# nicolas1805961/Cardiac-Segmentation-Optical-flow

Measured on AMD Instinct MI355X. Metric: cine frames/sec (seg+flow) at 256x256, higher is better.
Workload: dtype f16 MFMA hi/lo split, f32 accumulate (f32-class); 1 GPU; BASELINE config 4: joint seg+flow over 256x256x30 cine slices; Generic_UNet(32 base, 6 pools) 4-flip TTA on every frame + SegFlowGaussian(video.yaml) two-chunk ED-anchored recurrence + fused label warp; image=256x256

## Files before the change

cardiac-segmentation-optical-flow_amd/cineflow/_lib.py:

```python
import ctypes
import os

_HERE = os.path.dirname(os.path.abspath(__file__))
LIB_PATH = os.environ.get("CINEFLOW_LIB") or os.path.join(_HERE, "libcineflow_hip.so")


class CineflowLibraryError(RuntimeError):
    pass


class CineflowError(RuntimeError):
    pass


P = ctypes.c_void_p
I = ctypes.c_int
L = ctypes.c_long
F = ctypes.c_float
DBL = ctypes.c_double

SIGNATURES = {
    "cf_warp_bilinear_2d": [P, P, P, I, I, I, I, P],
    "cf_vecint_2d": [P, P, P, I, I, I, I, P],
    "cf_warp_labels_2d": [P, P, P, I, I, I, I, I, P],
# ... 41 lines not shown
    "cf_crop2d": [P, P, I, I, I, I, I, I, I, P],
    "cf_pad2d": [P, P, I, I, I, I, I, I, I, P],
    "cf_tta_accumulate": [P, P, I, I, I, I, I, I, F, P],
    "cf_flip2d": [P, P, I, I, I, I, I, P],
    "cf_tile_accumulate": [P, P, P, P, I, I, I, I, I, I, I, P],
    "cf_tile_finalize": [P, P, P, P, I, I, I, P],
    "cf_tile_gather": [P, P, P, I, I, I, I, I, I, I, P],
    "cf_tile_merge": [P, P, P, P, I, I, I, I, I, I, P, I, P, I, P],
    "cf_tta_accumulate_3d": [P, P, I, I, I, I, I, I, I, I, F, P],
    "cf_flip3d": [P, P, I, I, I, I, I, I, I, P],
    "cf_tile_accumulate_3d": [P, P, P, P, I, I, I, I, I, I, I, I, I, I, P],
    "cf_argmax_channels": [P, P, I, I, I, P],
    "cf_resize3d": [P, P, I, I, I, I, I, I, I, I, I, I, P],
    "cf_cc_init": [P, P, L, P, I, P],
    "cf_cc_sweep": [P, I, I, I, P, P],
    "cf_cc_count": [P, P, L, P],
    "cf_cc_remove": [P, P, P, L, I, DBL, DBL, P],
    "cf_cc_label": [P, P, I, I, I, P, P],
    "cf_cc_sizes": [P, P, P, P, L, P, P, P, P],
    "cf_pp_confusion": [P, P, I, I, I, I, P, P, P, P, P, P, P, DBL, P, P, P, P],
    "cf_cc_apply": [P, P, L, I, I, I, P, P, P, P, P, P, DBL, P, P],
    "cf_conv2d_small_cin": [P, P, P, P, I, I, I, I, I, I, P, I, P],
    "cf_conv2d_small_cout": [P, P, P, P, P, I, I, I, I, I, P],
    "cf_nonzero_mask": [P, I, L, P, P],
    "cf_fill_holes": [P, P, P, I, I, I, I, P],
    "cf_mask_bbox": [P, I, I, I, P, P],
    "cf_spline3_resample_axis": [P, P, L, I, L, I, P],
    "cf_slab_minmax_chunks": [I, I, I, L],
    "cf_slab_minmax": [P, I, I, I, L, P, P, P],
    "cf_slab_clip_to_f32": [P, P, I, I, I, L, P, P],
    "cf_masked_moments": [P, P, L, I, F, F, P, P],
    "cf_normalize": [P, P, L, I, F, F, F, F, I, P],
    "cf_nan_to_zero": [P, L, P],
    "cf_assign_where_ge": [P, P, L, F, F, P],
    "cf_seg_outside_mask": [P, P, I, L, F, P],
    "cf_prev_stage_onehot": [P, I, I, I, P, I, I, I, P, I, P],
    "cf_ensemble_merge": [P, I, I, I, I, I, I, P, I, I, I, I, I, I, P, P, P],
    "cf_confusion_counts": [P, P, L, P, P],
    "cf_label_confusion": [P, P, L, I, P, P],
    "cf_surface_border": [P, I, I, I, I, P, P, P],
    "cf_surface_min_dist": [P, I, P, I, DBL, DBL, DBL, P, P],
    "cf_max_sum_nonneg": [P, L, P, P],
    "cf_region_stats": [P, P, L, I, P, P],
    "cf_spatial_gradient3d": [P, P, L, I, I, I, P],
    "cf_slab_abs_sum": [P, I, I, I, L, P, P],
    "cf_ssim_map": [P, P, I, I, I, DBL, DBL, DBL, P, P],
# ... 40 lines not shown
```

cardiac-segmentation-optical-flow_amd/cineflow/inference.py:

```python
import os

import numpy as np
import torch

from . import ops


def compute_steps_for_sliding_window(patch_size, image_size, step_size):
    assert all(i >= j for i, j in zip(image_size, patch_size)), "image size must be as large or larger than patch_size"
    assert 0 < step_size <= 1, "step_size must be larger than 0 and smaller or equal to 1"
    target = [i * step_size for i in patch_size]
    num_steps = [int(np.ceil((i - k) / j)) + 1 for i, j, k in zip(image_size, target, patch_size)]
    steps = []
    for dim in range(len(patch_size)):
        max_step_value = image_size[dim] - patch_size[dim]
        actual = max_step_value / (num_steps[dim] - 1) if num_steps[dim] > 1 else 99999999999
        steps.append([int(np.round(actual * i)) for i in range(num_steps[dim])])
    return steps


def get_gaussian(patch_size, sigma_scale=1.0 / 8):
    from scipy.ndimage import gaussian_filter
    tmp = np.zeros(patch_size)
    tmp[tuple(i // 2 for i in patch_size)] = 1
# ... 298 lines not shown
    key = str(dev)
    if key not in _side:
        _side[key] = torch.cuda.Stream(device=dev)
    return _side[key]


def predict_cine_slices(flow_net, seg_net, frames, ed_labels=None, do_mirroring=True, mirror_axes=(0, 1), seg_mixed_precision=False):
    T, B, _, H, W = frames.shape
    dev = frames.device
    seg_terms = 1 if seg_mixed_precision else 3
    side = None
    if TWO_STREAMS:
        side = _side_stream(dev)
        side.wait_stream(torch.cuda.current_stream(dev))
        with torch.cuda.stream(side), ops.conv_terms(seg_terms):
            probs = ensemble_predict_2d(seg_net, frames.reshape(T * B, 1, H, W), mirror_axes, do_mirroring)
            seg = ops.argmax_channels(probs).view(T, B, H, W)
    else:
        with ops.conv_terms(seg_terms):
            probs = ensemble_predict_2d(seg_net, frames.reshape(T * B, 1, H, W), mirror_axes, do_mirroring)
        seg = ops.argmax_channels(probs).view(T, B, H, W)
    flow = torch.zeros((T, B, 2, H, W), dtype=torch.float32, device=dev)
    o1, o2 = chunk_orders(T)
    ragged = len(o1) == len(o2) + 1 and len(o2) > 1 and RAGGED_CHUNKS and hasattr(flow_net, "_narrow") and not getattr(flow_net, "raft", False)
    if len(o1) == len(o2) and len(o1) > 1:
        xin = torch.cat([frames[o1], frames[o2]], dim=1)
        bf = flow_net(xin)["backward_flow"]
        for j, t in enumerate(o1[1:]):
            flow[t] = bf[j, :B]
        for j, t in enumerate(o2[1:]):
            flow[t] = bf[j, B:]
    elif ragged:
        o2p = o2 + [o2[-1]]
        xin = torch.cat([frames[o1], frames[o2p]], dim=1)
        bf = flow_net(xin, keep_from=len(o2), keep=B)["backward_flow"]
        for j, t in enumerate(o1[1:]):
            flow[t] = bf[j, :B]
        for j, t in enumerate(o2[1:]):
            flow[t] = bf[j, B:]
    else:
        for order in (o1, o2):
            if len(order) > 1:
                bf = flow_net(frames[order].contiguous())["backward_flow"]
                for j, t in enumerate(order[1:]):
                    flow[t] = bf[j]
    if side is not None:
        torch.cuda.current_stream(dev).wait_stream(side)
        probs.record_stream(torch.cuda.current_stream(dev))
        seg.record_stream(torch.cuda.current_stream(dev))
    if ed_labels is None:
        ed_labels = seg[0].contiguous()
    registered = ops.warp_labels(flow, ed_labels, flow_net.num_classes if hasattr(flow_net, "num_classes") else 4)
    return {"seg": seg, "softmax": probs.view(T, B, -1, H, W), "flow": flow, "registered": registered}
```

cardiac-segmentation-optical-flow_amd/cineflow/models.py:

```python
import copy

import numpy as np
import torch

from . import ops
from .convroute import PackedConv
from .nn import (Module, conv_norm, Conv2d, ConvTranspose2d, GroupNorm, Conv3d, ConvTranspose3d, InstanceNorm3d, ResidualLayer3D, ConvBlocks2DGroupLegacy, Encoder2D, Decoder2D, CrossAttentionLayer,
                 TransformerFlowEncoderSuccessiveNoEmb, ConvGRUCell, SpatialTransformer, VecInt)


class CorrVolume(Module):

    def __init__(self, radius, stride):
        super().__init__()
        self.radius, self.stride = radius, stride

    def forward(self, cur, prev):
        return ops.corr_volume(cur, prev, self.radius, self.stride)


class CorrBlock:

    def __init__(self, fmap1, fmap2, num_levels=4, radius=4):
        self.num_levels, self.radius = num_levels, radius
# ... 119 lines not shown
            self.query_encoder = Encoder2D(in_dims=in_q, extra_block=extra_block, **enc)
            self.cost_volume_encoder_list, self.cost_volume_computation_list = [], []
            for idx, (dim, nb) in enumerate(zip(out_encoder_dims, skip_co_depth)):
                self.cost_volume_computation_list.append(CorrVolume(radius=radius[idx], stride=stride[idx]))
                self.cost_volume_encoder_list.append(
                    ConvBlocks2DGroupLegacy((2 * radius[idx] + 1) ** 2, dim, 1, residual=residual))
                self.skip_co_reduction_list.append(ConvBlocks2DGroupLegacy(2 * dim, dim, nb, residual=residual))
        else:
            in_q[0] = 2
            self.query_encoder = Encoder2D(in_dims=in_q, extra_block=False, motion_appearance=True, **enc)
            for dim, nb in zip(out_encoder_dims, skip_co_depth):
                self.skip_co_reduction_list.append(ConvBlocks2DGroupLegacy(2 * dim, dim, nb, residual=residual))
        dec_in = in_dims[:]
        dec_in[0] = 4
        self.flow_decoder = Decoder2D(d_model=d_model, dot_multiplier=2, conv_depth=conv_depth[::-1], in_encoder_dims=dec_in[::-1],
                                      out_encoder_dims=out_encoder_dims[::-1], num_classes=2, nb_conv=nb_conv, residual=residual)
        self.gru_cell = ConvGRUCell(input_size=(self.H, self.W), input_dim=d_model, hidden_dim=d_model)
        self.reduce_transformer = ConvBlocks2DGroupLegacy(d_model * 2, d_model, 1, residual=residual)
        self.bottleneck1 = CrossAttentionLayer(d_model, bottleneck_heads, nb_layers, dim_feedforward)
        self.bottleneck2 = CrossAttentionLayer(d_model, bottleneck_heads, nb_layers, dim_feedforward)
        if raft:
            self.update_block = BasicUpdateBlock(hidden_dim=d_model // 2)

    def forward(self, x, keep_from=None, keep=None):
        if self.raft:
            assert keep_from is None, "ragged batches are built for the two recurrent dispatches only"
            return self.forward_multi_task_flow_deformable_raft(x)
        if self.motion_appearance:
            return self.forward_motion_appearance(x, keep_from, keep)
        return self.forward_multi_task_flow_deformable_cost_volume_transformer_cat(x, keep_from, keep)

    @staticmethod
    def _narrow(t, n):
        if isinstance(t, (list, tuple)):
            return [SegFlowGaussian._narrow(u, n) for u in t]
        return t[:n].contiguous()

    @staticmethod
    def _stack_flows(flows, B):
        if all(f.shape[0] == B for f in flows):
            return torch.stack(flows, dim=0)
        out = torch.zeros((len(flows), B) + tuple(flows[0].shape[1:]), dtype=flows[0].dtype, device=flows[0].device)
        for i, f in enumerate(flows):
            out[i, :f.shape[0]] = f
        return out

    def _step_tail(self, f1, f2, hidden, new_skips, cum, x0, xt):
        gru_in = self.reduce_transformer(f1, x2=f2)
        hidden = self.gru_cell(gru_in, hidden)
        flow = self.flow_decoder(hidden, new_skips)
        cum = ops.add(cum, flow)
        past_motion, past_skips = self.memory_encoder(ops.memory_input(x0, xt, cum))
        return hidden, cum, past_motion, past_skips

    def forward_motion_appearance(self, x, keep_from=None, keep=None):
        T, B, C, H, W = x.shape
        B_all = B
        dev = x.device
        cum = torch.zeros((B, 2, H, W), dtype=torch.float32, device=dev)
        hidden = torch.zeros((B, self.d_model, self.H, self.W), dtype=torch.float32, device=dev)
        past_motion, past_skips = self.memory_encoder(ops.memory_input(x[0], x[0], cum))
        pair = torch.empty((B, 2, H, W), dtype=torch.float32, device=dev)
        ops.copy_channels(x[0], 0, 1, dst=pair, dst_coff=0)
        ops.copy_channels(x[0], 0, 1, dst=pair, dst_coff=1)
        first_app, _, _ = self.query_encoder(pair)
        prev_app = first_app
        flows = []
        x0 = x[0]
        for t in range(1, T):
            xt, xp = x[t], x[t - 1]
            if keep_from is not None and t >= keep_from:
                if B != keep:
                    B = keep
                    cum, hidden, past_motion, past_skips, first_app, prev_app, x0 = self._narrow(
                        (cum, hidden, past_motion, past_skips, first_app, prev_app, x0), B)
                xt, xp = xt[:B], xp[:B]
            pair = torch.empty((B, 2, H, W), dtype=torch.float32, device=dev)
            ops.copy_channels(xt, 0, 1, dst=pair, dst_coff=0)
            ops.copy_channels(xp, 0, 1, dst=pair, dst_coff=1)
            cur_app, _cur_motion, skips = self.query_encoder(pair)
            new_skips = [self.skip_co_reduction_list[s](skips[s], x2=past_skips[s]) for s in range(self.num_stages)]
            f1 = self.bottleneck1(query=cur_app, key=prev_app, value=prev_app)
            f2 = self.bottleneck2(query=cur_app, key=first_app, value=past_motion)
            hidden, cum, past_motion, past_skips = self._step_tail(f1, f2, hidden, new_skips, cum, x0, xt)
            flows.append(cum)
            prev_app = cur_app
        return {"backward_flow": self._stack_flows(flows, B_all)}

    def forward_multi_task_flow_deformable_cost_volume_transformer_cat(self, x, keep_from=None, keep=None):
        T, B, C, H, W = x.shape
        B_all = B
        dev = x.device
        cum = torch.zeros((B, 2, H, W), dtype=torch.float32, device=dev)
        hidden = torch.zeros((B, self.d_model, self.H, self.W), dtype=torch.float32, device=dev)
        past_motion, past_skips = self.memory_encoder(ops.memory_input(x[0], x[0], cum))
        first_feat, first_skips = self.query_encoder(x[0])
        prev_feat, prev_skips = first_feat, first_skips
        flows = []
        x0 = x[0]
        for t in range(1, T):
            xt = x[t]
            if keep_from is not None and t >= keep_from:
                if B != keep:
                    B = keep
                    cum, hidden, past_motion, past_skips, first_feat, prev_feat, prev_skips, x0 = self._narrow(
                        (cum, hidden, past_motion, past_skips, first_feat, prev_feat, prev_skips, x0), B)
                xt = xt[:B].contiguous()
            cur_feat, cur_skips = self.query_encoder(xt)
            new_skips = []
            for s in range(self.num_stages):
                corr = self.cost_volume_computation_list[s](cur_skips[s], prev_skips[s])
                corr = self.cost_volume_encoder_list[s](corr)
                new_skips.append(self.skip_co_reduction_list[s](corr, x2=past_skips[s]))
            f1 = self.bottleneck1(query=cur_feat, key=prev_feat, value=prev_feat)
            f2 = self.bottleneck2(query=cur_feat, key=first_feat, value=past_motion)
            hidden, cum, past_motion, past_skips = self._step_tail(f1, f2, hidden, new_skips, cum, x0, xt)
            flows.append(cum)
            prev_feat, prev_skips = cur_feat, cur_skips
        return {"backward_flow": self._stack_flows(flows, B_all)}

    def forward_multi_task_flow_deformable_raft(self, x):
        T, B, C, H, W = x.shape
        dev = x.device
        half = self.d_model // 2
        flow_up = torch.zeros((B, 2, H, W), dtype=torch.float32, device=dev)
        cnet = self.memory_encoder(ops.memory_input(x[0], x[0], flow_up))[0]
        net = ops.copy_channels(cnet, 0, half, act="tanh")
        inp_motion = torch.empty((B, 2 * half, H // 8, W // 8), dtype=torch.float32, device=dev)
        ops.copy_channels(cnet, half, half, dst=inp_motion, dst_coff=0, act="relu")
        coords0 = coords_grid(B, H // 8, W // 8, dev)
        coords1 = coords_grid(B, H // 8, W // 8, dev)
        f1 = self.query_encoder(x[0])[0]
        out = []
        for t in range(1, T):
            f2 = self.query_encoder(x[t])[0]
            corr_fn = CorrBlock(f1, f2, radius=4)
            its = []
            for _ in range(self.raft_iters):
                corr = corr_fn(coords1)
# ... 358 lines not shown
```

cardiac-segmentation-optical-flow_amd/cineflow/nn.py:

```python
import math

import torch

from . import ops
from .convroute import OWN, PackedConv, PackedConvT, split_key


class Module:

    def __init__(self):
        object.__setattr__(self, "_shapes", {})
        object.__setattr__(self, "_p", {})

    def _param(self, name, shape):
        self._shapes[name] = tuple(int(s) for s in shape)

    def _children(self):
        for k, v in self.__dict__.items():
            if k.startswith("_"):
                continue
            if isinstance(v, Module):
                yield k, v
            elif isinstance(v, (list, tuple)):
                for i, m in enumerate(v):
# ... 329 lines not shown
        for b in self.convs:
            x = b(x)
        return x


class DoubleConv(Module):

    def __init__(self, in_dim, out_dim, residual, stride=1, kernel_size=3):
        super().__init__()
        self.conv1 = Conv2d(in_dim, out_dim, kernel_size, stride=stride, padding=1)
        self.norm1 = GroupNorm(8, out_dim)
        self.conv2 = Conv2d(out_dim, out_dim, kernel_size, padding=1)
        self.norm2 = GroupNorm(8, out_dim)
        self.residual = residual
        self.has_ds = bool(residual and (in_dim != out_dim or stride != 1))
        if self.has_ds:
            self.downsample = {0: Conv2d(in_dim, out_dim, 1, stride=stride), 1: GroupNorm(8, out_dim)}

    def _conv2(self, t_raw, ws1):
        B, C, H, W = t_raw.shape
        coef = ops.group_norm_coef(ws1, self.norm1._p["weight"], self.norm1._p["bias"], self.norm1.groups, B, C, H * W, self.norm1.eps)
        return self.conv2.prenorm(t_raw, coef, -1.0, stats_groups=self.norm2.groups)

    def forward(self, x, x2=None):
        kw1 = {} if x2 is None else {"x2": x2}
        t, ws1 = self.conv1(x, stats_groups=self.norm1.groups, **kw1)
        pre = ws1 is not None and ops.CONV_MODE == "f16s" and self.conv2.prenorm_ok(t)
        if pre:
            y2, ws2 = self._conv2(t, ws1)
            conv2 = lambda **k: self.norm2(y2, act="gelu", ws=ws2, **k)
        else:
            t = self.norm1(t, act="gelu", ws=ws1)
            conv2 = lambda **k: conv_norm(self.conv2, self.norm2, t, act="gelu", **k)
        if not self.residual:
            return conv2()
        if self.has_ds:
            kw = {} if x2 is None else {"x2": x2}
            r, ws_r = self.downsample[0](x, stats_groups=self.downsample[1].groups, **kw)
            return conv2(res=r, res_mode="after_act", res_norm=(ws_r, self.downsample[1]))
        assert x2 is None
        return conv2(res=x, res_mode="after_act")


class SingleConv(Module):

    def __init__(self, in_dim, out_dim, residual, stride=1, kernel_size=3):
        super().__init__()
        self.conv1 = Conv2d(in_dim, out_dim, kernel_size, stride=stride, padding=1)
        self.norm1 = GroupNorm(8, out_dim)
        self.residual = residual
        self.has_ds = bool(residual and (in_dim != out_dim or stride != 1))
        if self.has_ds:
            self.downsample = Conv2d(in_dim, out_dim, 1, stride=stride)

    def forward(self, x, x2=None):
        if not self.residual:
            return conv_norm(self.conv1, self.norm1, x, x2=x2, act="gelu")
        r = self.downsample(x, x2=x2) if self.has_ds else x
        return conv_norm(self.conv1, self.norm1, x, x2=x2, act="gelu", res=r, res_mode="before_act")


class ConvBlocks2DGroupLegacy(Module):

    def __init__(self, in_dim, out_dim, nb_blocks, stride=1, residual=False, kernel_size=3, nb_conv=2):
        super().__init__()
        dims = torch.linspace(in_dim, out_dim, nb_blocks + 1).int()
        dims[1:] = (torch.round(dims[1:] / 8) * 8).int()
        fn = DoubleConv if nb_conv == 2 else SingleConv
        self.blocks = [fn(in_dim=int(dims[i]), out_dim=int(dims[i + 1]), residual=residual, stride=stride) for i in range(nb_blocks)]

    def forward(self, x, x2=None):
        for i, b in enumerate(self.blocks):
            x = b(x, x2=x2) if i == 0 else b(x)
        return x


class PatchExpand2DGroup(Module):

    def __init__(self, in_dim, out_dim):
        super().__init__()
        self.up = {0: ConvTranspose2d(in_dim, out_dim), 1: GroupNorm(8, out_dim)}

    def forward(self, x):
        return conv_norm(self.up[0], self.up[1], x, act="gelu")


class PatchMerging2DGroup(Module):

    def __init__(self, in_dim, out_dim):
        super().__init__()
        self.reduction = {0: Conv2d(in_dim, out_dim, 3, stride=2, padding=1), 1: GroupNorm(8, out_dim)}

    def forward(self, x):
        return conv_norm(self.reduction[0], self.reduction[1], x, act="gelu")


class Encoder2D(Module):
# ... 24 lines not shown
            x = ds(x)
        if self.motion_appearance:
            return self.out_conv(x), x, skips
        if self.extra_block:
            x = self.out_conv(x)
        return x, skips


class Decoder2D(Module):

    def __init__(self, d_model, conv_depth, in_encoder_dims, out_encoder_dims, num_classes, dot_multiplier, nb_conv, residual):
        super().__init__()
        assert dot_multiplier == 2
        self.num_stages = len(conv_depth)
        self.layers, self.upsample_layers = [], []
        for i in range(self.num_stages):
            in_dim = d_model if i == 0 else in_encoder_dims[i - 1]
            self.upsample_layers.append(PatchExpand2DGroup(in_dim, out_encoder_dims[i]))
            self.layers.append(ConvBlocks2DGroupLegacy(out_encoder_dims[i] * 2, out_encoder_dims[i], conv_depth[i], nb_conv=nb_conv,
                                                       residual=residual))
        self.final_conv = Conv2d(out_encoder_dims[-1], num_classes, 3, padding=1)

    def forward(self, x, skips):
        for layer, up, skip in zip(self.layers, self.upsample_layers, reversed(skips)):
            x = layer(skip, x2=up(x))
        return self.final_conv(x)


_pos_cache = {}


def position_embedding_sine_2d(H, W, C, device, temperature=10000.0, scale=2 * math.pi):
    key = (H, W, C, str(device))
    if key not in _pos_cache:
        npf = C // 2
        y_embed = torch.arange(1, H + 1, dtype=torch.float32)[:, None].expand(H, W)
        x_embed = torch.arange(1, W + 1, dtype=torch.float32)[None, :].expand(H, W)
        eps = 1e-6
        y_embed = y_embed / (y_embed[-1:, :] + eps) * scale
        x_embed = x_embed / (x_embed[:, -1:] + eps) * scale
        dim_t = torch.arange(npf, dtype=torch.float32)
        dim_t = temperature ** (2 * (dim_t // 2) / npf)
        pos_x = x_embed[:, :, None] / dim_t
        pos_y = y_embed[:, :, None] / dim_t
        pos_x = torch.stack((pos_x[:, :, 0::2].sin(), pos_x[:, :, 1::2].cos()), dim=3).flatten(2)
        pos_y = torch.stack((pos_y[:, :, 0::2].sin(), pos_y[:, :, 1::2].cos()), dim=3).flatten(2)
        pos = torch.cat((pos_y, pos_x), dim=2).permute(2, 0, 1).reshape(1, C, H * W).contiguous()
        _pos_cache[key] = pos.to(device)
    return _pos_cache[key]
# ... 154 lines not shown
```

cardiac-segmentation-optical-flow_amd/cineflow/ops.py:

```python
import contextlib
import math
import os

import numpy as np
import torch

from ._lib import lib, check

ACT = {None: 0, "none": 0, "gelu": 1, "relu": 2, "lrelu": 3, "tanh": 4, "sigmoid": 5}
RES = {None: 0, "none": 0, "before_act": 1, "after_act": 2}
OP = {"add": 0, "sub": 1, "mul": 2}


def _stream():
    return torch.cuda.current_stream().cuda_stream


def _f32(t, name="tensor"):
    if not isinstance(t, torch.Tensor) or not t.is_cuda:
        raise TypeError("%s must be a CUDA/HIP tensor (cineflow has no CPU path)" % name)
    if t.dtype != torch.float32:
        raise TypeError("%s must be float32, got %s" % (name, t.dtype))
    if not t.is_contiguous():
        raise ValueError("%s must be contiguous" % name)
# ... 385 lines not shown
    B, Cin, H, W = x.shape
    cout, cin_w, K, K2 = weight.shape
    assert cin_w == Cin and K == K2
    out = torch.empty((B, cout, H, W), dtype=torch.float32, device=x.device)
    ws = torch.empty(2 * B * stats_groups, dtype=torch.float64, device=x.device) if stats_groups else None
    check(lib().cf_conv2d_small_cin(_f32(x), _f32(weight), _opt(bias), _f32(out), B, Cin, H, W, cout, K, None if ws is None else ws.data_ptr(),
                                    stats_groups or 0, _stream()), "cf_conv2d_small_cin")
    return (out, ws) if stats_groups else out


def small_cout_supported(cout, kh, kw, stride, pad):
    return cout <= 4 and (kh, kw, tuple(pad)) == (3, 3, (1, 1)) and stride == 1


def conv2d_small_cout(x, weight, bias, res=None):
    B, Cin, H, W = x.shape
    cout = weight.shape[0]
    assert tuple(weight.shape) == (cout, Cin, 3, 3)
    out = torch.empty((B, cout, H, W), dtype=torch.float32, device=x.device)
    if res is not None:
        assert res.shape == out.shape
    check(lib().cf_conv2d_small_cout(_f32(x), _f32(weight), _opt(bias), _opt(res), _f32(out), B, Cin, H, W, cout, _stream()), "cf_conv2d_small_cout")
    return out


def prenorm_ok(x, cout):
    B, C, H, W = x.shape
    return bool(CONV_MODE == "f16s" and x.data_ptr() % 16 == 0 and lib().cf_conv2d_f16s_prenorm_ok(B, C, H, W, cout) == 1)


def group_norm_coef(ws, gamma, beta, groups, B, C, HW, eps=1e-5):
    coef = torch.empty((B, 3, C), dtype=torch.float32, device=ws.device)
    check(lib().cf_group_norm_coef(ws.data_ptr(), _opt(gamma), _opt(beta), B, C, HW, groups, float(eps), _f32(coef), _stream()), "cf_group_norm_coef")
    return coef


def norm_head_ok(x, K):
    return x.dim() == 4 and K in (2, 4, 8) and (x.shape[2] * x.shape[3]) % 4 == 0 and x.shape[1] <= 1024 and x.is_contiguous()


def norm_head_1x1(x, coef, slope, w, bias=None):
    B, C, H, W = x.shape
    K = w.shape[0]
    w2 = w.reshape(K, C).contiguous()
    out = torch.empty((B, K, H, W), dtype=torch.float32, device=x.device)
    check(lib().cf_norm_head_1x1(_f32(x), _f32(coef), float(slope), _f32(w2), _opt(bias), _f32(out), B, C, H * W, K, _stream()), "cf_norm_head_1x1")
# ... 542 lines not shown
```

cardiac-segmentation-optical-flow_amd/csrc/conv_direct.hip:

```cpp
#include "common.h"
#include "conv.h"
#include "profile.h"

namespace cf {

template <int CIN, int KS, int PY>
__global__ void __launch_bounds__(256) conv_small_cin_kernel(const float* __restrict__ x, const float* __restrict__ w, const float* __restrict__ bias,
                                                             float* __restrict__ out, int H, int W, int Cout, int groups,
                                                             double* __restrict__ gn_ws) {
    constexpr int R = KS / 2;
    constexpr int NR = PY + 2 * R, NC = KS;
    __shared__ float red[64 * 2];
    const int tx = threadIdx.x & 63, ty = threadIdx.x >> 6;
    const int x0 = blockIdx.x * 64 + tx, y0 = (blockIdx.y * 4 + ty) * PY, b = blockIdx.z;
    const long HW = (long)H * W;
    const float* xb = x + (long)b * CIN * HW;
    float* ob = out + (long)b * Cout * HW;
    if (groups > 0) {
        for (int k = threadIdx.x; k < 2 * groups; k += 256) red[k] = 0.f;
        __syncthreads();
    }
    float in[CIN][NR][NC];
#pragma unroll
    for (int ci = 0; ci < CIN; ++ci)
// ... 91 lines not shown
#pragma unroll
            for (int c = 0; c < 3; ++c) in[r][c] = __builtin_bit_cast(float, __builtin_amdgcn_raw_buffer_load_b32(rs, off[r][c] + cofs, 0, 0));
#pragma unroll
        for (int co = 0; co < COUT; ++co) {
            const float* wc = w + ((long)co * Cin + ci) * 9;
#pragma unroll
            for (int ky = 0; ky < 3; ++ky)
#pragma unroll
                for (int kx = 0; kx < 3; ++kx) {
                    const float wv = wc[ky * 3 + kx];
#pragma unroll
                    for (int r = 0; r < PY; ++r) acc[co][r] = fmaf(wv, in[r + ky][kx], acc[co][r]);
                }
        }
    }
    if (x0 >= W) return;
#pragma unroll
    for (int co = 0; co < COUT; ++co)
#pragma unroll
        for (int r = 0; r < PY; ++r) {
            if (y0 + r >= H) continue;
            const long o = ((long)b * COUT + co) * HW + (long)(y0 + r) * W + x0;
            out[o] = res ? acc[co][r] + res[o] : acc[co][r];
        }
}

}

using namespace cf;

extern "C" int cf_conv2d_small_cin(const float* x, const float* weight, const float* bias, float* out, int B, int Cin, int H, int W, int Cout, int K,
                                   double* gn_ws, int gn_groups, void* stream) {
    CF_REQUIRE(x && weight && out && x != out, "null or aliased pointer");
    CF_REQUIRE(B > 0 && B < 65536 && H > 0 && W > 0 && Cout > 0, "bad shape B=%d H=%d W=%d Cout=%d", B, H, W, Cout);
    CF_REQUIRE((K == 3 || K == 1) && (Cin == 1 || Cin == 2 || Cin == 6), "built for Cin 1, 2, 6 and 3x3 (pad 1) / 1x1 kernels, got Cin=%d K=%d", Cin, K);
    CF_REQUIRE(!gn_ws || (gn_groups > 0 && gn_groups <= 64 && Cout % gn_groups == 0), "bad GroupNorm statistics request (groups <= 64 dividing Cout)");
    hipStream_t s = as_stream(stream);
    const int groups = gn_ws ? gn_groups : 0;
    if (gn_ws && hipMemsetAsync(gn_ws, 0, 2L * B * groups * sizeof(double), s) != hipSuccess) { set_error("cf_conv2d_small_cin: memset failed"); return CF_ERR_LAUNCH; }
    if (K == 3) {
        if (Cin == 1) launch_small_cin<1, 3, 8>(x, weight, bias, out, B, H, W, Cout, groups, gn_ws, s);
        else if (Cin == 2) launch_small_cin<2, 3, 4>(x, weight, bias, out, B, H, W, Cout, groups, gn_ws, s);
        else launch_small_cin<6, 3, 2>(x, weight, bias, out, B, H, W, Cout, groups, gn_ws, s);
    } else {
        if (Cin == 1) launch_small_cin<1, 1, 8>(x, weight, bias, out, B, H, W, Cout, groups, gn_ws, s);
        else if (Cin == 2) launch_small_cin<2, 1, 8>(x, weight, bias, out, B, H, W, Cout, groups, gn_ws, s);
// ... 8 lines not shown
    CF_REQUIRE(x && weight && out && x != out, "null or aliased pointer");
    CF_REQUIRE(B > 0 && B < 65536 && Cin > 0 && H > 0 && W > 0, "bad shape B=%d Cin=%d H=%d W=%d", B, Cin, H, W);
    CF_REQUIRE(Cout >= 1 && Cout <= 4, "built for 1..4 output channels, got %d", Cout);
    CF_REQUIRE((double)Cin * H * W * 4.0 < 2147483648.0, "one input sample must stay below 2 GiB (32-bit buffer offsets)");
    hipStream_t s = as_stream(stream);
    constexpr int PY = 8;
    dim3 grid((unsigned)((W + 63) / 64), (unsigned)((H + 4 * PY - 1) / (4 * PY)), (unsigned)B);
    hipEvent_t e0, e1;
    const double bytes = 4.0 * B * H * W * (Cin + Cout);
    const bool prof = profile_on() && profile_events(PK_CONV_SMALL_COUT, bytes, &e0, &e1);
#define CF_LAUNCH_SC(N)                                                                                                                          \
    if (prof) hipExtLaunchKernelGGL((conv3x3_small_cout_kernel<N, PY>), grid, dim3(256), 0, s, e0, e1, 0, x, weight, bias, res, out, Cin, H, W);   \
    else hipLaunchKernelGGL((conv3x3_small_cout_kernel<N, PY>), grid, dim3(256), 0, s, x, weight, bias, res, out, Cin, H, W)
    switch (Cout) {
        case 1: CF_LAUNCH_SC(1); break;
        case 2: CF_LAUNCH_SC(2); break;
        case 3: CF_LAUNCH_SC(3); break;
        default: CF_LAUNCH_SC(4); break;
    }
#undef CF_LAUNCH_SC
    CF_CHECK_LAUNCH();
    return CF_OK;
}
```

include/cineflow.h:

```cpp
#ifndef CINEFLOW_H
#define CINEFLOW_H

#include <stdint.h>

#ifdef __cplusplus
extern "C" {
#endif

#define CF_OK 0
#define CF_ERR_ARG (-1)
#define CF_ERR_LAUNCH (-2)

#define CF_ACT_NONE 0
#define CF_ACT_GELU 1
#define CF_ACT_RELU 2
#define CF_ACT_LRELU 3
#define CF_ACT_TANH 4
#define CF_ACT_SIGMOID 5

#define CF_RES_NONE 0
#define CF_RES_BEFORE_ACT 1
#define CF_RES_AFTER_ACT 2

const char* cf_last_error(void);
// ... 114 lines not shown
int cf_cc_init(const uint8_t* image, int* labels, long n, const uint8_t* classes, int nclasses, void* stream);
int cf_cc_sweep(int* labels, int D, int H, int W, int* changed, void* stream);
int cf_cc_count(const int* labels, int* counts, long n, void* stream);
int cf_cc_remove(uint8_t* image, const int* labels, const int* counts, long n, int max_count, double volume_per_voxel,
                 double min_valid, void* stream);

int cf_cc_label(const uint8_t* image, int* labels, int D, int H, int W, const uint8_t* region_of, void* stream);
int cf_cc_sizes(const int* labels, const uint8_t* image, const uint8_t* region_of, const uint8_t* alive, long n, int* counts,
                int* region_max, int* region_max_alive, void* stream);
int cf_pp_confusion(const uint8_t* pred, const uint8_t* gt, int D, int H, int W, int K, const int* labels_fg, const int* counts_fg,
                    const int* max_fg, const int* labels_cls, const int* counts_cls, const int* max_cls, const int* max_cls_alive,
                    double volume_per_voxel, const double* min_valid, const int* z_skip, unsigned long long* out, void* stream);
int cf_cc_apply(const uint8_t* src, uint8_t* dst, long n, int K, int do_fg, int class_bits, const int* labels_fg, const int* counts_fg,
                const int* max_fg, const int* labels_cls, const int* counts_cls, const int* max_cls, double volume_per_voxel,
                const double* min_valid, void* stream);

int cf_resize3d(const float* src, float* dst, int N, int X, int Y, int Z, int X2, int Y2, int Z2, int linear_x, int linear_y,
                int linear_z, void* stream);

int cf_conv2d_small_cin(const float* x, const float* weight, const float* bias, float* out, int B, int Cin, int H, int W, int Cout, int K,
                        double* gn_ws, int gn_groups, void* stream);
int cf_conv2d_small_cout(const float* x, const float* weight, const float* bias, const float* res, float* out, int B, int Cin, int H, int W,
                         int Cout, void* stream);

int cf_nonzero_mask(const float* data, int C, long V, uint8_t* mask, void* stream);
int cf_fill_holes(uint8_t* mask, const int* labels, int* touch, int D, int H, int W, int ndim, void* stream);
int cf_mask_bbox(const uint8_t* mask, int D, int H, int W, int* bbox, void* stream);
int cf_spline3_resample_axis(const double* src, double* dst, long outer, int n, long inner, int m, void* stream);
int cf_slab_minmax_chunks(int C, int A, int S, long B);
int cf_slab_minmax(const double* x, int C, int A, int S, long B, double* minmax, double* partial, void* stream);
int cf_slab_clip_to_f32(const double* y, float* out, int C, int A, int S, long B, const double* minmax, void* stream);
int cf_masked_moments(const float* x, const float* seg, long n, int use_range, float lo, float hi, double* out3, void* stream);
int cf_normalize(float* x, const float* seg, long n, int clip, float lo, float hi, float sub, float div, int zero_outside, void* stream);
int cf_nan_to_zero(float* x, long n, void* stream);
int cf_assign_where_ge(float* dst, const float* src, long n, float thr, float value, void* stream);
int cf_seg_outside_mask(float* seg, const uint8_t* mask, int C, long V, float label, void* stream);
int cf_prev_stage_onehot(const uint8_t* seg, int X, int Y, int Z, float* dst, int X2, int Y2, int Z2, const uint8_t* classes,
                         int n_classes, void* stream);
int cf_ensemble_merge(const void* const* members, int n_members, int dtype, int K, int Z, int Y, int X, uint8_t* seg, int Zf, int Yf, int Xf,
                      int z0, int y0, int x0, void* mean, const uint8_t* order, void* stream);

int cf_confusion_counts(const uint8_t* test, const uint8_t* reference, long n, unsigned long long* counts3, void* stream);
int cf_label_confusion(const uint8_t* test, const uint8_t* reference, long n, int K, unsigned long long* hist, void* stream);
int cf_surface_border(const uint8_t* mask, int D, int H, int W, int ndim, int* coords, int* count, void* stream);
int cf_surface_min_dist(const int* a, int na, const int* b, int nb, double sz, double sy, double sx, double* dist, void* stream);
int cf_max_sum_nonneg(const double* x, long n, double* out2, void* stream);
// ... 20 lines not shown
```

Measured before the change: 782.3 frames/s.

## Share ED-frame encoding across chunks, fuse stem and final-conv norm, skip last memory step

Several independent changes. The ED anchor frame is now encoded once for both recurrence chunks and the result duplicated, instead of being encoded twice. The memory encoder is skipped on the final timestep, and it runs on a narrowed batch for the ragged chunk. A new fused stem kernel computes the 3x3 conv, the 1x1 downsample and both GroupNorm statistics in one pass. A new small-Cout conv kernel applies norm2, the residual norm, GELU and the add while computing the final 3x3 conv, so the normalized activation is never written out. Together these cut redundant encoder work and kernel launches, at the cost of more special-case code paths.

After: 797.1 frames/s, median of 6. 1.02x the previous value.

```diff
diff --git a/cardiac-segmentation-optical-flow_amd/cineflow/_lib.py b/cardiac-segmentation-optical-flow_amd/cineflow/_lib.py
--- a/cardiac-segmentation-optical-flow_amd/cineflow/_lib.py
+++ b/cardiac-segmentation-optical-flow_amd/cineflow/_lib.py
@@ -87,6 +87,10 @@
     "cf_cc_apply": [P, P, L, I, I, I, P, P, P, P, P, P, DBL, P, P],
     "cf_conv2d_small_cin": [P, P, P, P, I, I, I, I, I, I, P, I, P],
     "cf_conv2d_small_cout": [P, P, P, P, P, I, I, I, I, I, P],
+    "cf_conv2d_small_cout_norm2_ok": [I, I, I, I, I],
+    "cf_conv2d_small_cout_norm2": [P, P, P, P, P, P, P, I, I, I, I, I, P],
+    "cf_stem_block_ok": [I, I, I, I, I, I],
+    "cf_stem_block": [P, P, P, P, P, P, P, I, I, I, I, I, P, P, I, P],
     "cf_nonzero_mask": [P, I, L, P, P],
     "cf_fill_holes": [P, P, P, I, I, I, I, P],
     "cf_mask_bbox": [P, I, I, I, P, P],
diff --git a/cardiac-segmentation-optical-flow_amd/cineflow/inference.py b/cardiac-segmentation-optical-flow_amd/cineflow/inference.py
--- a/cardiac-segmentation-optical-flow_amd/cineflow/inference.py
+++ b/cardiac-segmentation-optical-flow_amd/cineflow/inference.py
@@ -344,10 +344,11 @@
         seg = ops.argmax_channels(probs).view(T, B, H, W)
     flow = torch.zeros((T, B, 2, H, W), dtype=torch.float32, device=dev)
     o1, o2 = chunk_orders(T)
+    shared = {"shared_first": B} if hasattr(flow_net, "_narrow") and not getattr(flow_net, "raft", False) else {}
     ragged = len(o1) == len(o2) + 1 and len(o2) > 1 and RAGGED_CHUNKS and hasattr(flow_net, "_narrow") and not getattr(flow_net, "raft", False)
     if len(o1) == len(o2) and len(o1) > 1:
         xin = torch.cat([frames[o1], frames[o2]], dim=1)
-        bf = flow_net(xin)["backward_flow"]
+        bf = flow_net(xin, **shared)["backward_flow"]
         for j, t in enumerate(o1[1:]):
             flow[t] = bf[j, :B]
         for j, t in enumerate(o2[1:]):
@@ -355,7 +356,7 @@
     elif ragged:
         o2p = o2 + [o2[-1]]
         xin = torch.cat([frames[o1], frames[o2p]], dim=1)
-        bf = flow_net(xin, keep_from=len(o2), keep=B)["backward_flow"]
+        bf = flow_net(xin, keep_from=len(o2), keep=B, **shared)["backward_flow"]
         for j, t in enumerate(o1[1:]):
             flow[t] = bf[j, :B]
         for j, t in enumerate(o2[1:]):
diff --git a/cardiac-segmentation-optical-flow_amd/cineflow/models.py b/cardiac-segmentation-optical-flow_amd/cineflow/models.py
--- a/cardiac-segmentation-optical-flow_amd/cineflow/models.py
+++ b/cardiac-segmentation-optical-flow_amd/cineflow/models.py
@@ -165,13 +165,14 @@
         if raft:
             self.update_block = BasicUpdateBlock(hidden_dim=d_model // 2)
 
-    def forward(self, x, keep_from=None, keep=None):
+    def forward(self, x, keep_from=None, keep=None, shared_first=None):
         if self.raft:
-            assert keep_from is None, "ragged batches are built for the two recurrent dispatches only"
+            assert keep_from is None and shared_first is None, "ragged / shared-ED batches are built for the two recurrent dispatches only"
             return self.forward_multi_task_flow_deformable_raft(x)
+        assert shared_first is None or x.shape[1] == 2 * shared_first, "shared_first=n describes a batch of 2n sequences"
         if self.motion_appearance:
-            return self.forward_motion_appearance(x, keep_from, keep)
-        return self.forward_multi_task_flow_deformable_cost_volume_transformer_cat(x, keep_from, keep)
+            return self.forward_motion_appearance(x, keep_from, keep, shared_first)
+        return self.forward_multi_task_flow_deformable_cost_volume_transformer_cat(x, keep_from, keep, shared_first)
 
     @staticmethod
     def _narrow(t, n):
@@ -188,25 +189,43 @@
             out[i, :f.shape[0]] = f
         return out
 
-    def _step_tail(self, f1, f2, hidden, new_skips, cum, x0, xt):
+    @staticmethod
+    def _twice(t):
+        if isinstance(t, (list, tuple)):
+            return [SegFlowGaussian._twice(u) for u in t]
+        return t.repeat(2, 1, 1, 1)
+
+    def _step_tail(self, f1, f2, hidden, new_skips, cum, x0, xt, last=False, go_on=None):
         gru_in = self.reduce_transformer(f1, x2=f2)
         hidden = self.gru_cell(gru_in, hidden)
         flow = self.flow_decoder(hidden, new_skips)
         cum = ops.add(cum, flow)
-        past_motion, past_skips = self.memory_encoder(ops.memory_input(x0, xt, cum))
+        if last:
+            return hidden, cum, None, None
+        if go_on is not None and go_on < cum.shape[0]:
+            past_motion, past_skips = self.memory_encoder(ops.memory_input(*self._narrow((x0, xt, cum), go_on)))
+        else:
+            past_motion, past_skips = self.memory_encoder(ops.memory_input(x0, xt, cum))
         return hidden, cum, past_motion, past_skips
 
-    def forward_motion_appearance(self, x, keep_from=None, keep=None):
+    def _tail_flags(self, t, T, B, keep_from, keep):
+        return dict(last=t == T - 1, go_on=keep if (keep_from is not None and t == keep_from - 1 and B != keep) else None)
+
+    def forward_motion_appearance(self, x, keep_from=None, keep=None, shared_first=None):
         T, B, C, H, W = x.shape
         B_all = B
         dev = x.device
         cum = torch.zeros((B, 2, H, W), dtype=torch.float32, device=dev)
         hidden = torch.zeros((B, self.d_model, self.H, self.W), dtype=torch.float32, device=dev)
-        past_motion, past_skips = self.memory_encoder(ops.memory_input(x[0], x[0], cum))
-        pair = torch.empty((B, 2, H, W), dtype=torch.float32, device=dev)
-        ops.copy_channels(x[0], 0, 1, dst=pair, dst_coff=0)
-        ops.copy_channels(x[0], 0, 1, dst=pair, dst_coff=1)
+        n0 = shared_first or B
+        e0, c0 = self._narrow((x[0], cum), n0)
+        past_motion, past_skips = self.memory_encoder(ops.memory_input(e0, e0, c0))
+        pair = torch.empty((n0, 2, H, W), dtype=torch.float32, device=dev)
+        ops.copy_channels(e0, 0, 1, dst=pair, dst_coff=0)
+        ops.copy_channels(e0, 0, 1, dst=pair, dst_coff=1)
         first_app, _, _ = self.query_encoder(pair)
+        if shared_first:
+            past_motion, past_skips, first_app = self._twice((past_motion, past_skips, first_app))
         prev_app = first_app
         flows = []
         x0 = x[0]
@@ -225,19 +244,23 @@
             new_skips = [self.skip_co_reduction_list[s](skips[s], x2=past_skips[s]) for s in range(self.num_stages)]
             f1 = self.bottleneck1(query=cur_app, key=prev_app, value=prev_app)
             f2 = self.bottleneck2(query=cur_app, key=first_app, value=past_motion)
-            hidden, cum, past_motion, past_skips = self._step_tail(f1, f2, hidden, new_skips, cum, x0, xt)
+            hidden, cum, past_motion, past_skips = self._step_tail(f1, f2, hidden, new_skips, cum, x0, xt, **self._tail_flags(t, T, B, keep_from, keep))
             flows.append(cum)
             prev_app = cur_app
         return {"backward_flow": self._stack_flows(flows, B_all)}
 
-    def forward_multi_task_flow_deformable_cost_volume_transformer_cat(self, x, keep_from=None, keep=None):
+    def forward_multi_task_flow_deformable_cost_volume_transformer_cat(self, x, keep_from=None, keep=None, shared_first=None):
         T, B, C, H, W = x.shape
         B_all = B
         dev = x.device
         cum = torch.zeros((B, 2, H, W), dtype=torch.float32, device=dev)
         hidden = torch.zeros((B, self.d_model, self.H, self.W), dtype=torch.float32, device=dev)
-        past_motion, past_skips = self.memory_encoder(ops.memory_input(x[0], x[0], cum))
-        first_feat, first_skips = self.query_encoder(x[0])
+        n0 = shared_first or B
+        e0, c0 = self._narrow((x[0], cum), n0)
+        past_motion, past_skips = self.memory_encoder(ops.memory_input(e0, e0, c0))
+        first_feat, first_skips = self.query_encoder(e0)
+        if shared_first:
+            past_motion, past_skips, first_feat, first_skips = self._twice((past_motion, past_skips, first_feat, first_skips))
         prev_feat, prev_skips = first_feat, first_skips
         flows = []
         x0 = x[0]
@@ -257,7 +280,7 @@
                 new_skips.append(self.skip_co_reduction_list[s](corr, x2=past_skips[s]))
             f1 = self.bottleneck1(query=cur_feat, key=prev_feat, value=prev_feat)
             f2 = self.bottleneck2(query=cur_feat, key=first_feat, value=past_motion)
-            hidden, cum, past_motion, past_skips = self._step_tail(f1, f2, hidden, new_skips, cum, x0, xt)
+            hidden, cum, past_motion, past_skips = self._step_tail(f1, f2, hidden, new_skips, cum, x0, xt, **self._tail_flags(t, T, B, keep_from, keep))
             flows.append(cum)
             prev_feat, prev_skips = cur_feat, cur_skips
         return {"backward_flow": self._stack_flows(flows, B_all)}
diff --git a/cardiac-segmentation-optical-flow_amd/cineflow/nn.py b/cardiac-segmentation-optical-flow_amd/cineflow/nn.py
--- a/cardiac-segmentation-optical-flow_amd/cineflow/nn.py
+++ b/cardiac-segmentation-optical-flow_amd/cineflow/nn.py
@@ -375,24 +375,40 @@
         coef = ops.group_norm_coef(ws1, self.norm1._p["weight"], self.norm1._p["bias"], self.norm1.groups, B, C, H * W, self.norm1.eps)
         return self.conv2.prenorm(t_raw, coef, -1.0, stats_groups=self.norm2.groups)
 
-    def forward(self, x, x2=None):
+    def _stem_ok(self, x, x2):
+        c1 = self.conv1
+        return (x2 is None and self.has_ds and c1.sub is None and c1.stride == 1 and c1.cin <= 8 and c1.ks == (3, 3) and c1.pad == (1, 1)
+                and self.downsample[1].groups == self.norm1.groups and ops.stem_block_ok(x, c1.cout, self.norm1.groups))
+
+    def forward(self, x, x2=None, defer_last=None):
         kw1 = {} if x2 is None else {"x2": x2}
-        t, ws1 = self.conv1(x, stats_groups=self.norm1.groups, **kw1)
+        r = ws_r = None
+        if self._stem_ok(x, x2):
+            ds = self.downsample[0]
+            t, ws1, r, ws_r = ops.stem_block(x, self.conv1._p["weight"], self.conv1._p.get("bias"), ds._p["weight"], ds._p.get("bias"), self.norm1.groups)
+        else:
+            t, ws1 = self.conv1(x, stats_groups=self.norm1.groups, **kw1)
         pre = ws1 is not None and ops.CONV_MODE == "f16s" and self.conv2.prenorm_ok(t)
+        y2 = ws2 = None
         if pre:
             y2, ws2 = self._conv2(t, ws1)
             conv2 = lambda **k: self.norm2(y2, act="gelu", ws=ws2, **k)
         else:
             t = self.norm1(t, act="gelu", ws=ws1)
             conv2 = lambda **k: conv_norm(self.conv2, self.norm2, t, act="gelu", **k)
+        done = (lambda out: out) if defer_last is None else (lambda out: (out, None))
         if not self.residual:
-            return conv2()
+            return done(conv2())
         if self.has_ds:
-            kw = {} if x2 is None else {"x2": x2}
-            r, ws_r = self.downsample[0](x, stats_groups=self.downsample[1].groups, **kw)
-            return conv2(res=r, res_mode="after_act", res_norm=(ws_r, self.downsample[1]))
+            if r is None:
+                kw = {} if x2 is None else {"x2": x2}
+                r, ws_r = self.downsample[0](x, stats_groups=self.downsample[1].groups, **kw)
+            if (defer_last is not None and ws2 is not None and ws_r is not None and defer_last.sub is None
+                    and ops.small_cout_norm2_ok(y2, defer_last.cout, defer_last.ks[0], defer_last.ks[1], defer_last.stride, defer_last.pad)):
+                return None, ((y2, ws2, self.norm2), (r, ws_r, self.downsample[1]))
+            return done(conv2(res=r, res_mode="after_act", res_norm=(ws_r, self.downsample[1])))
         assert x2 is None
-        return conv2(res=x, res_mode="after_act")
+        return done(conv2(res=x, res_mode="after_act"))
 
 
 class SingleConv(Module):
@@ -422,10 +438,15 @@
         fn = DoubleConv if nb_conv == 2 else SingleConv
         self.blocks = [fn(in_dim=int(dims[i]), out_dim=int(dims[i + 1]), residual=residual, stride=stride) for i in range(nb_blocks)]
 
-    def forward(self, x, x2=None):
+    def forward(self, x, x2=None, defer_last=None):
+        pending = None
         for i, b in enumerate(self.blocks):
-            x = b(x, x2=x2) if i == 0 else b(x)
-        return x
+            kw = {"x2": x2} if i == 0 else {}
+            if defer_last is not None and i == len(self.blocks) - 1 and isinstance(b, DoubleConv):
+                x, pending = b(x, defer_last=defer_last, **kw)
+            else:
+                x = b(x, **kw)
+        return (x, pending) if defer_last is not None else x
 
 
 class PatchExpand2DGroup(Module):
@@ -496,9 +517,20 @@
         self.final_conv = Conv2d(out_encoder_dims[-1], num_classes, 3, padding=1)
 
     def forward(self, x, skips):
-        for layer, up, skip in zip(self.layers, self.upsample_layers, reversed(skips)):
-            x = layer(skip, x2=up(x))
-        return self.final_conv(x)
+        pending = None
+        for i, (layer, up, skip) in enumerate(zip(self.layers, self.upsample_layers, reversed(skips))):
+            if i == self.num_stages - 1:
+                x, pending = layer(skip, x2=up(x), defer_last=self.final_conv)
+            else:
+                x = layer(skip, x2=up(x))
+        if pending is None:
+            return self.final_conv(x)
+        coefs = []
+        for raw, ws, norm in pending:
+            B, C, H, W = raw.shape
+            coefs.append(ops.group_norm_coef(ws, norm._p["weight"], norm._p["bias"], norm.groups, B, C, H * W, norm.eps))
+        (y2, _, _), (r, _, _) = pending
+        return ops.conv2d_small_cout_norm2(y2, coefs[0], r, coefs[1], self.final_conv._p["weight"], self.final_conv._p.get("bias"))
 
 
 _pos_cache = {}
diff --git a/cardiac-segmentation-optical-flow_amd/cineflow/ops.py b/cardiac-segmentation-optical-flow_amd/cineflow/ops.py
--- a/cardiac-segmentation-optical-flow_amd/cineflow/ops.py
+++ b/cardiac-segmentation-optical-flow_amd/cineflow/ops.py
@@ -431,6 +431,40 @@
         assert res.shape == out.shape
     check(lib().cf_conv2d_small_cout(_f32(x), _f32(weight), _opt(bias), _opt(res), _f32(out), B, Cin, H, W, cout, _stream()), "cf_conv2d_small_cout")
     return out
+
+
+def small_cout_norm2_ok(y2, cout, kh, kw, stride, pad):
+    B, C, H, W = y2.shape
+    return bool(CONV_MODE == "f16s" and small_cout_supported(cout, kh, kw, stride, pad) and lib().cf_conv2d_small_cout_norm2_ok(B, C, H, W, cout) == 1)
+
+
+def conv2d_small_cout_norm2(y2, coef2, r, coefr, weight, bias):
+    B, Cin, H, W = y2.shape
+    cout = weight.shape[0]
+    assert tuple(weight.shape) == (cout, Cin, 3, 3) and r.shape == y2.shape
+    assert tuple(coef2.shape) == (B, 3, Cin) and tuple(coefr.shape) == (B, 3, Cin)
+    out = torch.empty((B, cout, H, W), dtype=torch.float32, device=y2.device)
+    check(lib().cf_conv2d_small_cout_norm2(_f32(y2), _f32(coef2), _f32(r), _f32(coefr), _f32(weight), _opt(bias), _f32(out), B, Cin, H, W, cout,
+                                           _stream()), "cf_conv2d_small_cout_norm2")
+    return out
+
+
+def stem_block_ok(x, cout, groups):
+    B, Cin, H, W = x.shape
+    return bool(CONV_MODE == "f16s" and lib().cf_stem_block_ok(B, Cin, H, W, cout, groups) == 1)
+
+
+def stem_block(x, w3, b3, w1, b1, groups):
+    B, Cin, H, W = x.shape
+    cout = w3.shape[0]
+    assert tuple(w3.shape) == (cout, Cin, 3, 3) and tuple(w1.shape) == (cout, Cin, 1, 1)
+    y = torch.empty((B, cout, H, W), dtype=torch.float32, device=x.device)
+    r = torch.empty_like(y)
+    ws = _zeroed_stats_ws(4 * B * groups, x.device)
+    ws_y, ws_r = ws[:2 * B * groups], ws[2 * B * groups:]
+    check(lib().cf_stem_block(_f32(x), _f32(w3), _opt(b3), _f32(w1), _opt(b1), _f32(y), _f32(r), B, Cin, H, W, cout, ws_y.data_ptr(), ws_r.data_ptr(),
+                              -groups, _stream()), "cf_stem_block")
+    return y, ws_y, r, ws_r
 
 
 def prenorm_ok(x, cout):
diff --git a/cardiac-segmentation-optical-flow_amd/csrc/conv_direct.hip b/cardiac-segmentation-optical-flow_amd/csrc/conv_direct.hip
--- a/cardiac-segmentation-optical-flow_amd/csrc/conv_direct.hip
+++ b/cardiac-segmentation-optical-flow_amd/csrc/conv_direct.hip
@@ -137,6 +137,93 @@
             if (y0 + r >= H) continue;
             const long o = ((long)b * COUT + co) * HW + (long)(y0 + r) * W + x0;
             out[o] = res ? acc[co][r] + res[o] : acc[co][r];
+        }
+}
+
+template <int COUT, int PY>
+__global__ void __launch_bounds__(256, 4) conv3x3_small_cout_norm2_kernel(const float* __restrict__ y2, const float* __restrict__ coef2,
+                                                                          const float* __restrict__ r, const float* __restrict__ coefr,
+                                                                          const float* __restrict__ w, const float* __restrict__ bias,
+                                                                          float* __restrict__ out, int Cin, int H, int W) {
+    constexpr int NR = PY + 2;
+    constexpr int TH = 4 * PY + 2, TW = 66, TN = TH * TW, NS = (TN + 255) / 256;
+    constexpr unsigned OOB = 0x80000000u;
+    __shared__ float tile[2][TN];
+    const int tx = threadIdx.x & 63, ty = threadIdx.x >> 6;
+    const int bx0 = blockIdx.x * 64, by0 = blockIdx.y * 4 * PY, b = blockIdx.z;
+    const int x0 = bx0 + tx, y0 = by0 + ty * PY;
+    const long HW = (long)H * W;
+    const int bytes = (int)((long)Cin * HW * 4);
+    const __amdgpu_buffer_rsrc_t rs2 = __builtin_amdgcn_make_buffer_rsrc(const_cast<float*>(y2 + (long)b * Cin * HW), 0, bytes, 0x00020000);
+    const __amdgpu_buffer_rsrc_t rsr = __builtin_amdgcn_make_buffer_rsrc(const_cast<float*>(r + (long)b * Cin * HW), 0, bytes, 0x00020000);
+    unsigned off[NS];
+#pragma unroll
+    for (int k = 0; k < NS; ++k) {
+        const int e = (int)threadIdx.x + 256 * k, tr = e / TW, tc = e - tr * TW;
+        const int yy = by0 + tr - 1, xx = bx0 + tc - 1;
+        off[k] = (e < TN && yy >= 0 && yy < H && xx >= 0 && xx < W) ? (unsigned)(yy * W + xx) * 4u : OOB;
+    }
+    float acc[COUT][PY];
+#pragma unroll
+    for (int co = 0; co < COUT; ++co)
+#pragma unroll
+        for (int rr = 0; rr < PY; ++rr) acc[co][rr] = bias ? bias[co] : 0.f;
+    const unsigned HW4 = (unsigned)HW * 4u;
+    const float* c2 = coef2 + (long)b * 3 * Cin;
+    const float* cr = coefr + (long)b * 3 * Cin;
+    float a[NS], q[NS];
+#pragma unroll
+    for (int k = 0; k < NS; ++k) {
+        a[k] = __builtin_bit_cast(float, __builtin_amdgcn_raw_buffer_load_b32(rs2, off[k], 0, 0));
+        q[k] = __builtin_bit_cast(float, __builtin_amdgcn_raw_buffer_load_b32(rsr, off[k], 0, 0));
+    }
+#pragma unroll 1
+    for (int ci = 0; ci < Cin; ++ci) {
+        float* t = tile[ci & 1];
+        const float m2 = c2[ci], s2 = c2[Cin + ci], b2 = c2[2 * Cin + ci];
+        const float mr = cr[ci], sr = cr[Cin + ci], br = cr[2 * Cin + ci];
+#pragma unroll
+        for (int k = 0; k < NS; ++k) {
+            const int e = (int)threadIdx.x + 256 * k;
+            float v = (a[k] - m2) * s2 + b2;
+            v = gelu_as(v);
+            v += (q[k] - mr) * sr + br;
+            if (e < TN) t[e] = off[k] != OOB ? v : 0.f;
+        }
+        if (ci + 1 < Cin) {
+            const unsigned cofs = (unsigned)(ci + 1) * HW4;
+#pragma unroll
+            for (int k = 0; k < NS; ++k) {
+                a[k] = __builtin_bit_cast(float, __builtin_amdgcn_raw_buffer_load_b32(rs2, off[k] + cofs, 0, 0));
+                q[k] = __builtin_bit_cast(float, __builtin_amdgcn_raw_buffer_load_b32(rsr, off[k] + cofs, 0, 0));
+            }
+        }
+        __syncthreads();
+        float in[NR][3];
+#pragma unroll
+        for (int rr = 0; rr < NR; ++rr)
+#pragma unroll
+            for (int c = 0; c < 3; ++c) in[rr][c] = t[(ty * PY + rr) * TW + tx + c];
+#pragma unroll
+        for (int co = 0; co < COUT; ++co) {
+            const float* wc = w + ((long)co * Cin + ci) * 9;
+#pragma unroll
+            for (int ky = 0; ky < 3; ++ky)
+#pragma unroll
+                for (int kx = 0; kx < 3; ++kx) {
+                    const float wv = wc[ky * 3 + kx];
+#pragma unroll
+                    for (int rr = 0; rr < PY; ++rr) acc[co][rr] = fmaf(wv, in[rr + ky][kx], acc[co][rr]);
+                }
+        }
+    }
+    if (x0 >= W) return;
+#pragma unroll
+    for (int co = 0; co < COUT; ++co)
+#pragma unroll
+        for (int rr = 0; rr < PY; ++rr) {
+            if (y0 + rr >= H) continue;
+            out[((long)b * COUT + co) * HW + (long)(y0 + rr) * W + x0] = acc[co][rr];
         }
 }
 
@@ -191,3 +278,26 @@
     CF_CHECK_LAUNCH();
     return CF_OK;
 }
+
+extern "C" int cf_conv2d_small_cout_norm2_ok(int B, int Cin, int H, int W, int Cout) {
+    return B > 0 && B < 65536 && Cin > 0 && H > 0 && W > 0 && Cout >= 1 && Cout <= 4 && (H + 31) / 32 < 65536 && (double)Cin * H * W * 4.0 < 2147483648.0 ? 1 : 0;
+}
+
+extern "C" int cf_conv2d_small_cout_norm2(const float* y2, const float* coef2, const float* r, const float* coefr, const float* weight, const float* bias,
+                                          float* out, int B, int Cin, int H, int W, int Cout, void* stream) {
+    CF_REQUIRE(y2 && coef2 && r && coefr && weight && out && y2 != out && r != out, "null or aliased pointer");
+    CF_REQUIRE(cf_conv2d_small_cout_norm2_ok(B, Cin, H, W, Cout) == 1,
+               "built for 1..4 output channels and input samples below 2 GiB (32-bit buffer offsets): B=%d Cin=%d H=%d W=%d Cout=%d", B, Cin, H, W, Cout);
+    hipStream_t s = as_stream(stream);
+    constexpr int PY = 8;
+    dim3 grid((unsigned)((W + 63) / 64), (unsigned)((H + 4 * PY - 1) / (4 * PY)), (unsigned)B);
+    const double bytes = 4.0 * B * H * W * (2.0 * Cin + Cout);
+    switch (Cout) {
+        case 1: launch_profiled(PK_CONV_SMALL_COUT, bytes, conv3x3_small_cout_norm2_kernel<1, PY>, grid, dim3(256), s, y2, coef2, r, coefr, weight, bias, out, Cin, H, W); break;
+        case 2: launch_profiled(PK_CONV_SMALL_COUT, bytes, conv3x3_small_cout_norm2_kernel<2, PY>, grid, dim3(256), s, y2, coef2, r, coefr, weight, bias, out, Cin, H, W); break;
+        case 3: launch_profiled(PK_CONV_SMALL_COUT, bytes, conv3x3_small_cout_norm2_kernel<3, PY>, grid, dim3(256), s, y2, coef2, r, coefr, weight, bias, out, Cin, H, W); break;
+        default: launch_profiled(PK_CONV_SMALL_COUT, bytes, conv3x3_small_cout_norm2_kernel<4, PY>, grid, dim3(256), s, y2, coef2, r, coefr, weight, bias, out, Cin, H, W); break;
+    }
+    CF_CHECK_LAUNCH();
+    return CF_OK;
+}
diff --git a/cardiac-segmentation-optical-flow_amd/csrc/conv_stem.hip b/cardiac-segmentation-optical-flow_amd/csrc/conv_stem.hip
--- /dev/null
+++ b/cardiac-segmentation-optical-flow_amd/csrc/conv_stem.hip
@@ -0,0 +1,125 @@
+#include "common.h"
+#include "conv.h"
+#include "profile.h"
+
+namespace cf {
+
+template <int CIN, int PY>
+__global__ void __launch_bounds__(256) stem_block_kernel(const float* __restrict__ x, const float* __restrict__ w3, const float* __restrict__ b3,
+                                                         const float* __restrict__ w1, const float* __restrict__ b1, float* __restrict__ y,
+                                                         float* __restrict__ r, int H, int W, int Cout, int groups,
+                                                         double* __restrict__ ws_y, double* __restrict__ ws_r) {
+    constexpr int NR = PY + 2;
+    __shared__ float red[2][64 * 2];
+    const int tx = threadIdx.x & 63, ty = threadIdx.x >> 6;
+    const int x0 = blockIdx.x * 64 + tx, y0 = (blockIdx.y * 4 + ty) * PY, b = blockIdx.z;
+    const long HW = (long)H * W;
+    const float* xb = x + (long)b * CIN * HW;
+    float* yb = y + (long)b * Cout * HW;
+    float* rb = r + (long)b * Cout * HW;
+    for (int k = threadIdx.x; k < 2 * groups; k += 256) red[0][k] = red[1][k] = 0.f;
+    __syncthreads();
+    float in[CIN][NR][3];
+#pragma unroll
+    for (int ci = 0; ci < CIN; ++ci)
+#pragma unroll
+        for (int rr = 0; rr < NR; ++rr)
+#pragma unroll
+            for (int c = 0; c < 3; ++c) {
+                const int yy = y0 + rr - 1, xx = x0 + c - 1;
+                in[ci][rr][c] = (yy >= 0 && yy < H && xx >= 0 && xx < W) ? xb[ci * HW + (long)yy * W + xx] : 0.f;
+            }
+    bool ok[PY];
+#pragma unroll
+    for (int rr = 0; rr < PY; ++rr) ok[rr] = x0 < W && y0 + rr < H;
+    const int cpg = Cout / groups;
+    for (int g = 0; g < groups; ++g) {
+        float ys = 0.f, yq = 0.f, rs = 0.f, rq = 0.f;
+        for (int c = 0; c < cpg; ++c) {
+            const int co = g * cpg + c;
+            const float* w3c = w3 + (long)co * CIN * 9;
+            const float* w1c = w1 + (long)co * CIN;
+            const float bv3 = b3 ? b3[co] : 0.f, bv1 = b1 ? b1[co] : 0.f;
+            float wr[CIN * 9], wp[CIN];
+#pragma unroll
+            for (int k = 0; k < CIN * 9; ++k) wr[k] = w3c[k];
+#pragma unroll
+            for (int k = 0; k < CIN; ++k) wp[k] = w1c[k];
+#pragma unroll
+            for (int rr = 0; rr < PY; ++rr) {
+                float acc = bv3, pacc = bv1;
+#pragma unroll
+                for (int ci = 0; ci < CIN; ++ci)
+#pragma unroll
+                    for (int ky = 0; ky < 3; ++ky)
+#pragma unroll
+                        for (int kx = 0; kx < 3; ++kx) acc = fmaf(wr[(ci * 3 + ky) * 3 + kx], in[ci][rr + ky][kx], acc);
+#pragma unroll
+                for (int ci = 0; ci < CIN; ++ci) pacc = fmaf(wp[ci], in[ci][rr + 1][1], pacc);
+                if (ok[rr]) {
+                    const long o = (long)co * HW + (long)(y0 + rr) * W + x0;
+                    yb[o] = acc;
+                    rb[o] = pacc;
+                    ys += acc;
+                    yq += acc * acc;
+                    rs += pacc;
+                    rq += pacc * pacc;
+                }
+            }
+        }
+        for (int o = 32; o > 0; o >>= 1) {
+            ys += __shfl_xor(ys, o, 64);
+            yq += __shfl_xor(yq, o, 64);
+            rs += __shfl_xor(rs, o, 64);
+            rq += __shfl_xor(rq, o, 64);
+        }
+        if (tx == 0) {
+            atomicAdd(&red[0][2 * g], ys);
+            atomicAdd(&red[0][2 * g + 1], yq);
+            atomicAdd(&red[1][2 * g], rs);
+            atomicAdd(&red[1][2 * g + 1], rq);
+        }
+    }
+    __syncthreads();
+    for (int k = threadIdx.x; k < 4 * groups; k += 256) {
+        const int m = k >= 2 * groups, j = k - m * 2 * groups;
+        atomicAdd(&(m ? ws_r : ws_y)[2L * b * groups + j], (double)red[m][j]);
+    }
+}
+
+template <int CIN, int PY>
+static void launch_stem_block(const float* x, const float* w3, const float* b3, const float* w1, const float* b1, float* y, float* r, int B, int H,
+                              int W, int Cout, int groups, double* ws_y, double* ws_r, hipStream_t s) {
+    dim3 grid((unsigned)((W + 63) / 64), (unsigned)((H + 4 * PY - 1) / (4 * PY)), (unsigned)B);
+    hipLaunchKernelGGL((stem_block_kernel<CIN, PY>), grid, dim3(256), 0, s, x, w3, b3, w1, b1, y, r, H, W, Cout, groups, ws_y, ws_r);
+}
+
+}
+
+using namespace cf;
+
+extern "C" int cf_stem_block_ok(int B, int Cin, int H, int W, int Cout, int gn_groups) {
+    return (Cin == 1 || Cin == 6) && B > 0 && B < 65536 && H > 0 && W > 0 && (H + 7) / 8 < 65536 && Cout > 0 && gn_groups > 0 && gn_groups <= 64 &&
+                   Cout % gn_groups == 0 && (double)Cout * H * W < 2147483648.0
+               ? 1 : 0;
+}
+
+extern "C" int cf_stem_block(const float* x, const float* w3, const float* b3, const float* w1, const float* b1, float* y, float* r, int B, int Cin,
+                             int H, int W, int Cout, double* ws_y, double* ws_r, int gn_groups, void* stream) {
+    CF_REQUIRE(x && w3 && w1 && y && r && ws_y && ws_r, "null pointer");
+    CF_REQUIRE(x != y && x != r && y != r && ws_y != ws_r, "aliased pointers");
+    const int groups = gn_groups < 0 ? -gn_groups : gn_groups;
+    CF_REQUIRE(cf_stem_block_ok(B, Cin, H, W, Cout, groups) == 1,
+               "built for Cin 1 or 6, <= 64 statistics groups dividing Cout, one output sample below 2^31 elements: B=%d Cin=%d H=%d W=%d Cout=%d groups=%d", B,
+               Cin, H, W, Cout, groups);
+    hipStream_t s = as_stream(stream);
+    if (gn_groups > 0 && (hipMemsetAsync(ws_y, 0, 2L * B * groups * sizeof(double), s) != hipSuccess ||
+                          hipMemsetAsync(ws_r, 0, 2L * B * groups * sizeof(double), s) != hipSuccess)) {
+        set_error("cf_stem_block: memset failed");
+        return CF_ERR_LAUNCH;
+    }
+    if (Cin == 1) launch_stem_block<1, 8>(x, w3, b3, w1, b1, y, r, B, H, W, Cout, groups, ws_y, ws_r, s);
+    else launch_stem_block<6, 4>(x, w3, b3, w1, b1, y, r, B, H, W, Cout, groups, ws_y, ws_r, s);
+    CF_CHECK_LAUNCH();
+    return CF_OK;
+}
diff --git a/include/cineflow.h b/include/cineflow.h
--- a/include/cineflow.h
+++ b/include/cineflow.h
@@ -160,6 +160,12 @@
                         double* gn_ws, int gn_groups, void* stream);
 int cf_conv2d_small_cout(const float* x, const float* weight, const float* bias, const float* res, float* out, int B, int Cin, int H, int W,
                          int Cout, void* stream);
+int cf_conv2d_small_cout_norm2_ok(int B, int Cin, int H, int W, int Cout);
+int cf_conv2d_small_cout_norm2(const float* y2, const float* coef2, const float* r, const float* coefr, const float* weight, const float* bias,
+                               float* out, int B, int Cin, int H, int W, int Cout, void* stream);
+int cf_stem_block_ok(int B, int Cin, int H, int W, int Cout, int gn_groups);
+int cf_stem_block(const float* x, const float* w3, const float* b3, const float* w1, const float* b1, float* y, float* r, int B, int Cin,
+                  int H, int W, int Cout, double* ws_y, double* ws_r, int gn_groups, void* stream);
 
 int cf_nonzero_mask(const float* data, int C, long V, uint8_t* mask, void* stream);
 int cf_fill_holes(uint8_t* mask, const int* labels, int* touch, int D, int H, int W, int ndim, void* stream);
```
